# LanDiff/LanDiff

Measured on AMD Instinct MI355X. Metric: end-to-end frames/sec, 49f 480x720 @50 steps, higher is better.
Workload: dtype bf16; 1 GPU; LanDiff 5B full pipeline, single prompt per GPU, 49f 480x720, 50 sampler steps (VPSDE DPM-Solver++(2M), DynamicCFG), bf16, random-init weights at true shapes; frames=49, height=480, width=720, sampler_steps=50, llm_steps=1244, parallelism=dp1 over prompts, RCCL all_gather of uint8 frames only

## Files before the change

### landiff_amd/csrc/ld_llm.hip

```cpp
#include "ld_common.h"
#include "ld_llm_dev.h"
#include <stdio.h>
#include <stdlib.h>
#include "../../include/landiff_hip.h"

namespace {

constexpr int MAXB = 4;

struct GemvParams {
  const void* x;
  const void* W;
  const void* W2;
  const bf16_t* bias;
  const void* resid;
  void* out;
  int B, N, K;
  long ldx, ldo, ldr;
  int x_f32, w_f32, out_f32;
  int in_act, act;
  const float* norm_w;
  float norm_eps;
  ChainSync cs;
};
// ... 215 lines not shown
  constexpr int NV = R * B * (GATED ? 2 : 1), V = ceil_pow2(NV), LOGV = ilog2(V);
  constexpr int XAUX = CHAIN ? 16 : 0;
  __shared__ float red[2][4][V];
  __shared__ float ssq[4][B];

  const int tid = threadIdx.x, lane = tid & 63, wave = tid >> 6;
  const int nchunk = p.K >> 3;
  const int er = tid / B, eb = tid - er * B;

  u32x4_t wn[R][J], w2n[GATED ? R : 1][J];
  uint32_t e_bias_n = 0u, e_res_n = 0u;
  auto request = [&](int batch) {
    const int n0 = batch * R;
#pragma unroll
    for (int r = 0; r < R; ++r) {
      const long row = (n0 + r < p.N) ? n0 + r : p.N - 1;
#pragma unroll
      for (int j = 0; j < J; ++j) {
        const int c = j * 256 + tid;
        wn[r][j] = (u32x4_t){0u, 0u, 0u, 0u};
        if (c < nchunk) wn[r][j] = __builtin_nontemporal_load((const u32x4_t*)((const bf16_t*)p.W + row * p.K + c * 8));
        if (GATED) {
          w2n[r][j] = (u32x4_t){0u, 0u, 0u, 0u};
          if (c < nchunk) w2n[r][j] = __builtin_nontemporal_load((const u32x4_t*)((const bf16_t*)p.W2 + row * p.K + c * 8));
        }
      }
    }
    const int en = n0 + er;
    if (tid < R * B && en < p.N) {
      if (p.bias) e_bias_n = p.bias[en];
      if (p.resid) {
        if (CHAIN) e_res_n = __hip_atomic_load((const bf16_t*)p.resid + eb * p.ldr + en, __ATOMIC_RELAXED, __HIP_MEMORY_SCOPE_AGENT);
        else e_res_n = p.out_f32 ? ((const uint32_t*)p.resid)[eb * p.ldr + en] : (uint32_t)((const bf16_t*)p.resid)[eb * p.ldr + en];
      }
    }
  };

  u32x4_t xq[B][J];
  f32x4_t g0[NORM ? J : 1], g1[NORM ? J : 1];
  int batch = blockIdx.x;
  if (CHAIN) {
    request(batch);
    chain_wait(p.cs, tid);
  }
#pragma unroll
  for (int b = 0; b < B; ++b) {
    const __amdgpu_buffer_rsrc_t rx = __builtin_amdgcn_make_buffer_rsrc((void*)((const bf16_t*)p.x + b * p.ldx), 0, p.K * 2, 0x00020000);
#pragma unroll
    for (int j = 0; j < J; ++j) xq[b][j] = __builtin_amdgcn_raw_buffer_load_b128(rx, (j * 256 + tid) * 16, 0, XAUX);
  }
  if (NORM) {
    const __amdgpu_buffer_rsrc_t rg = __builtin_amdgcn_make_buffer_rsrc((void*)p.norm_w, 0, p.K * 4, 0x00020000);
#pragma unroll
    for (int j = 0; j < J; ++j) {
      const u32x4_t a = __builtin_amdgcn_raw_buffer_load_b128(rg, (j * 256 + tid) * 32, 0, 0);
      const u32x4_t b = __builtin_amdgcn_raw_buffer_load_b128(rg, (j * 256 + tid) * 32 + 16, 0, 0);
      g0[j] = __builtin_bit_cast(f32x4_t, a); g1[j] = __builtin_bit_cast(f32x4_t, b);
    }
  }
  if (!CHAIN) request(batch);

  if (NORM) {
#pragma unroll
    for (int b = 0; b < B; ++b) {
      const float ss = wave_sum(chunks_sumsq<J>(xq[b]));
      if (lane == 0) ssq[wave][b] = ss;
    }
    __syncthreads();
#pragma unroll
    for (int b = 0; b < B; ++b) {
      const float r1 = rsqrtf((ssq[0][b] + ssq[1][b] + ssq[2][b] + ssq[3][b]) / (float)p.K + p.norm_eps);
#pragma unroll
      for (int j = 0; j < J; ++j) {
        if (j * 256 + tid < nchunk) {
          const u32x4_t a = xq[b][j];
          xq[b][j] = (u32x4_t){pack_bf16x2(bf_lo(a[0]) * r1 * g0[j][0], bf_hi(a[0]) * r1 * g0[j][1]),
                               pack_bf16x2(bf_lo(a[1]) * r1 * g0[j][2], bf_hi(a[1]) * r1 * g0[j][3]),
                               pack_bf16x2(bf_lo(a[2]) * r1 * g1[j][0], bf_hi(a[2]) * r1 * g1[j][1]),
                               pack_bf16x2(bf_lo(a[3]) * r1 * g1[j][2], bf_hi(a[3]) * r1 * g1[j][3])};
        }
      }
    }
  }

  int par = 0;
#pragma unroll 1
  for (; batch < nbatch; batch += gridDim.x, par ^= 1) {
    u32x4_t w[R][J], w2[GATED ? R : 1][J];
#pragma unroll
    for (int r = 0; r < R; ++r)
#pragma unroll
      for (int j = 0; j < J; ++j) { w[r][j] = wn[r][j]; if (GATED) w2[r][j] = w2n[r][j]; }
    const uint32_t e_bias_raw = e_bias_n, e_res_raw = e_res_n;
    if (batch + (int)gridDim.x < nbatch) request(batch + gridDim.x);

    float v[V];
#pragma unroll
    for (int i = 0; i < V; ++i) v[i] = 0.f;
#pragma unroll
    for (int r = 0; r < R; ++r)
#pragma unroll
      for (int j = 0; j < J; ++j)
#pragma unroll
        for (int b = 0; b < B; ++b)
#pragma unroll
          for (int e = 0; e < 4; ++e) {
            v[r * B + b] = dot2_bf16(w[r][j][e], xq[b][j][e], v[r * B + b]);
            if (GATED) v[R * B + r * B + b] = dot2_bf16(w2[r][j][e], xq[b][j][e], v[R * B + r * B + b]);
          }
    wave_sum_multi<V>(v, lane);
    if ((lane & ((64 >> LOGV) - 1)) == 0) red[par][wave][lane >> (6 - LOGV)] = v[0];
    __syncthreads();
    const int en = batch * R + er;
    if (tid < R * B && en < p.N) {
      const float(&rd)[4][V] = red[par];
      float a = rd[0][tid] + rd[1][tid] + rd[2][tid] + rd[3][tid];
      const float e_bias = bf2f((bf16_t)e_bias_raw), e_res = p.out_f32 ? __uint_as_float(e_res_raw) : bf2f((bf16_t)e_res_raw);
      if (p.bias) a += e_bias;
      a = rbf(a);
      if (p.act) a = rbf(apply_act(p.act, a));
      if (GATED) a = rbf(a * rbf(rd[0][R * B + tid] + rd[1][R * B + tid] + rd[2][R * B + tid] + rd[3][R * B + tid]));
      if (p.resid) a = p.out_f32 ? e_res + a : rbf(e_res + a);
      if (CHAIN) __hip_atomic_store((bf16_t*)p.out + eb * p.ldo + en, f2bf(a), __ATOMIC_RELAXED, __HIP_MEMORY_SCOPE_AGENT);
      else if (p.out_f32) ((float*)p.out)[eb * p.ldo + en] = a;
      else ((bf16_t*)p.out)[eb * p.ldo + en] = f2bf(a);
    }
  }
  if (CHAIN) chain_arrive(p.cs, tid, blockIdx.x);
}

__global__ __launch_bounds__(256) void ld_rmsnorm_kernel(const bf16_t* x, const float* w, bf16_t* out,
                                                         int rows, int D, float eps) {
  const int lane = threadIdx.x & 63;
  const int r = blockIdx.x * 4 + (threadIdx.x >> 6);
  if (r >= rows) return;
  const bf16_t* xr = x + (long)r * D;
  float ss = 0.f;
  for (int c = lane; c < (D >> 3); c += 64) {
    const u32x4_t a = *(const u32x4_t*)(xr + c * 8);
#pragma unroll
    for (int e = 0; e < 4; ++e) { const float lo = bf_lo(a[e]), hi = bf_hi(a[e]); ss += lo * lo + hi * hi; }
  }
  ss = wave_sum(ss);
  const float rs = rsqrtf(ss / (float)D + eps);
  for (int c = lane; c < (D >> 3); c += 64) {
    const u32x4_t a = *(const u32x4_t*)(xr + c * 8);
    const f32x4_t w0 = *(const f32x4_t*)(w + c * 8), w1 = *(const f32x4_t*)(w + c * 8 + 4);
    float v[8];
#pragma unroll
    for (int e = 0; e < 4; ++e) { v[2 * e] = bf_lo(a[e]) * rs; v[2 * e + 1] = bf_hi(a[e]) * rs; }
    u32x4_t o;
    o[0] = pack_bf16x2(v[0] * w0[0], v[1] * w0[1]); o[1] = pack_bf16x2(v[2] * w0[2], v[3] * w0[3]);
    o[2] = pack_bf16x2(v[4] * w1[0], v[5] * w1[1]); o[3] = pack_bf16x2(v[6] * w1[2], v[7] * w1[3]);
    *(u32x4_t*)(out + (long)r * D + c * 8) = o;
  }
}

__global__ __launch_bounds__(256) void ld_ln_f32out_kernel(const bf16_t* x, long ldx, const float* w, const float* b,
                                                           float* out, int rows, int D, float eps) {
  const int lane = threadIdx.x & 63;
  const int r = blockIdx.x * 4 + (threadIdx.x >> 6);
  if (r >= rows) return;
  const bf16_t* xr = x + (long)r * ldx;
  float s = 0.f, ss = 0.f;
  for (int i = lane; i < D; i += 64) { const float v = bf2f(xr[i]); s += v; }
  s = wave_sum(s);
  const float mean = s / (float)D;
  for (int i = lane; i < D; i += 64) { const float d = bf2f(xr[i]) - mean; ss += d * d; }
  ss = wave_sum(ss);
  const float rs = rsqrtf(ss / (float)D + eps);
  for (int i = lane; i < D; i += 64) out[(long)r * D + i] = (bf2f(xr[i]) - mean) * rs * w[i] + b[i];
}

__global__ __launch_bounds__(256) void ld_ln_f32out_reg_kernel(const bf16_t* x, long ldx, const float* w, const float* b,
                                                               float* out, int rows, int D, float eps) {
  const int lane = threadIdx.x & 63;
  const int r = blockIdx.x * 4 + (threadIdx.x >> 6);
  if (r >= rows) return;
  const bf16_t* xr = x + (long)r * ldx;
  const int nchunk = D >> 3;
  float v[8][8];
  float s = 0.f, ss = 0.f;
#pragma unroll
  for (int k = 0; k < 8; ++k) {
    const int c = lane + 64 * k;
    u32x4_t a = (u32x4_t){0u, 0u, 0u, 0u};
    if (c < nchunk) a = *(const u32x4_t*)(xr + c * 8);
#pragma unroll
    for (int e = 0; e < 4; ++e) { v[k][2 * e] = bf_lo(a[e]); v[k][2 * e + 1] = bf_hi(a[e]); s += v[k][2 * e] + v[k][2 * e + 1]; }
  }
  s = wave_sum(s);
  const float mean = s / (float)D;
#pragma unroll
  for (int k = 0; k < 8; ++k) {
    if (lane + 64 * k < nchunk) {
#pragma unroll
      for (int e = 0; e < 8; ++e) { const float d = v[k][e] - mean; ss += d * d; }
    }
  }
  ss = wave_sum(ss);
  const float rs = rsqrtf(ss / (float)D + eps);
#pragma unroll
  for (int k = 0; k < 8; ++k) {
    const int c = lane + 64 * k;
    if (c < nchunk) {
      const f32x4_t w0 = *(const f32x4_t*)(w + c * 8), w1 = *(const f32x4_t*)(w + c * 8 + 4);
      const f32x4_t b0 = *(const f32x4_t*)(b + c * 8), b1 = *(const f32x4_t*)(b + c * 8 + 4);
      f32x4_t o0, o1;
#pragma unroll
      for (int e = 0; e < 4; ++e) { o0[e] = (v[k][e] - mean) * rs * w0[e] + b0[e]; o1[e] = (v[k][4 + e] - mean) * rs * w1[e] + b1[e]; }
      *(f32x4_t*)(out + (long)r * D + c * 8) = o0;
      *(f32x4_t*)(out + (long)r * D + c * 8 + 4) = o1;
    }
  }
}

__global__ void ld_rope_append_kernel(const bf16_t* qkv, const float* cos_t, const float* sin_t, const int* pos_ptr,
                                      bf16_t* q_out, bf16_t* kc, bf16_t* vc, int B, int m, int H, int Lmax) {
  const int D = 128;
  const int idx = blockIdx.x * blockDim.x + threadIdx.x;
  const int total = B * m * H * (D / 2);
  if (idx >= total) return;
  const int pr = idx % (D / 2);
  const int h = (idx / (D / 2)) % H;
  const int j = (idx / (D / 2) / H) % m;
  const int b = idx / (D / 2) / H / m;
  const int pos = *pos_ptr + j;
  const float c = cos_t[pos * (D / 2) + pr], s = sin_t[pos * (D / 2) + pr];
  const long base = (((long)(b * m + j) * 3) * H + h) * D + 2 * pr;
  const long hd = (long)H * D;
  const float qa = bf2f(qkv[base]), qb = bf2f(qkv[base + 1]);
  const float ka = bf2f(qkv[base + hd]), kb = bf2f(qkv[base + hd + 1]);
  const long qo = ((long)(b * m + j) * H + h) * D + 2 * pr;
  q_out[qo] = f2bf(qa * c - qb * s);
  q_out[qo + 1] = f2bf(qa * s + qb * c);
  const long co = (((long)b * Lmax + pos) * H + h) * D + 2 * pr;
  kc[co] = f2bf(ka * c - kb * s);
  kc[co + 1] = f2bf(ka * s + kb * c);
  vc[co] = qkv[base + 2 * hd];
  vc[co + 1] = qkv[base + 2 * hd + 1];
}

__global__ __launch_bounds__(256) void ld_kv_attn_kernel(const bf16_t* q, const bf16_t* kc, const bf16_t* vc,
                                                         const int* pos_ptr, bf16_t* out, int B, int m, int H, int Lmax) {
  extern __shared__ float sc[];
  const int D = 128;
  const int bh = blockIdx.x, j = blockIdx.y;
  const int b = bh / H, h = bh - b * H;
  const int L = *pos_ptr + j + 1;
  const int tid = threadIdx.x, lane = tid & 63, wave = tid >> 6;
  const bf16_t* qv = q + ((long)(b * m + j) * H + h) * D;
  const int sub = lane & 15, kq = lane >> 4;
  float qreg[8];
  {
    const u32x4_t a = *(const u32x4_t*)(qv + sub * 8);
#pragma unroll
    for (int e = 0; e < 4; ++e) { qreg[2 * e] = bf_lo(a[e]); qreg[2 * e + 1] = bf_hi(a[e]); }
  }
  const float inv_sqrt_d = 0.08838834764831845f;
  float lmax = -3.0e38f;
  for (int k0 = wave * 4; k0 < L; k0 += 16) {
    const int key = k0 + kq;
    float d = 0.f;
    if (key < L) {
      const u32x4_t a = *(const u32x4_t*)(kc + (((long)b * Lmax + key) * H + h) * D + sub * 8);
#pragma unroll
      for (int e = 0; e < 4; ++e) { d = fmaf(qreg[2 * e], bf_lo(a[e]), d); d = fmaf(qreg[2 * e + 1], bf_hi(a[e]), d); }
    }
    d += __shfl_xor(d, 1, 64); d += __shfl_xor(d, 2, 64); d += __shfl_xor(d, 4, 64); d += __shfl_xor(d, 8, 64);
    if (key < L) {
      const float s = rbf(rbf(d) * inv_sqrt_d);
      if (sub == 0) sc[key] = s;
      lmax = fmaxf(lmax, s);
    }
  }
  float* red = sc + Lmax;
  lmax = wave_max(lmax);
  if (lane == 0) red[wave] = lmax;
  __syncthreads();
  const float mx = fmaxf(fmaxf(red[0], red[1]), fmaxf(red[2], red[3]));
  float lsum = 0.f;
  for (int k = tid; k < L; k += 256) { const float e = __expf(sc[k] - mx); sc[k] = e; lsum += e; }
  lsum = wave_sum(lsum);
  __syncthreads();
  if (lane == 0) red[4 + wave] = lsum;
  __syncthreads();
  const float inv = 1.0f / (red[4] + red[5] + red[6] + red[7]);
  const int d = tid & 127, par = tid >> 7;
  float acc = 0.f;
  for (int k = par; k < L; k += 2) {
    const float pk = rbf(sc[k] * inv);
    acc = fmaf(pk, bf2f(vc[(((long)b * Lmax + k) * H + h) * D + d]), acc);
  }
  float* part = red + 8;
  part[par * 128 + d] = acc;
  __syncthreads();
  if (tid < 128) out[((long)(b * m + j) * H + h) * D + tid] = f2bf(part[tid] + part[128 + tid]);
}

__device__ __forceinline__ float ld_agent(const float* p) { return __hip_atomic_load(p, __ATOMIC_RELAXED, __HIP_MEMORY_SCOPE_AGENT); }
__device__ __forceinline__ void st_agent(float* p, float v) { __hip_atomic_store(p, v, __ATOMIC_RELAXED, __HIP_MEMORY_SCOPE_AGENT); }

template <bool CHAIN>
__global__ __launch_bounds__(256, CHAIN ? 2 : 1) void ld_kv_attn_split_kernel(const bf16_t* q, const bf16_t* qkv, const float* cos_t,
                                                               const float* sin_t, bf16_t* kc, bf16_t* vc,
                                                               const int* pos_ptr, int pos_value, float* ws, unsigned* counters,
                                                               bf16_t* out, int B, int H, int Lmax, int nsplit, KvSplitRule rule,
                                                               ChainSync cs) {
  __shared__ float red[8 + 4 * 128];
  __shared__ int is_last;
  const int D = 128;
  const int bh = blockIdx.x, sp = blockIdx.y;
  const int b = bh / H, h = bh - b * H;
  const int L = (pos_value >= 0 ? pos_value : *pos_ptr) + 1;
  const int ns = kv_eff_splits(L, nsplit, rule);
  const int tid = threadIdx.x, lane = tid & 63, wave = tid >> 6;
  if (sp >= ns) {
    if (CHAIN) { chain_wait(cs, tid); chain_arrive(cs, tid, blockIdx.y * gridDim.x + blockIdx.x); }
    return;
  }
  const int chunk = (L + ns - 1) / ns;
  const int k_begin = sp * chunk, k_end = min(L, k_begin + chunk);
  const int n = max(0, k_end - k_begin);
  const int sub = lane & 15, kq = lane >> 4;
  float* out_ws = ws + ((long)bh * nsplit + sp) * (D + 2);
  bf16_t* direct = (ns == 1 && !CHAIN) ? out + (long)bh * D : nullptr;
  KvRows rows;
  if (CHAIN) {
    if (n > 0) kv_rows_request(rows, kc, vc, (long)b * Lmax + k_begin, H, h, n, wave, kq, sub);
    chain_wait(cs, tid);
  }
  if (n == 0) {
    if (tid < D) st_agent(out_ws + 2 + tid, 0.f);
    if (tid == 0) { st_agent(out_ws, -3.0e38f); st_agent(out_ws + 1, 0.f); }
  } else {
    u32x4_t a_q = (u32x4_t){0u, 0u, 0u, 0u}, a_k = a_q, a_v = a_q;
    float cs_[4] = {0.f, 0.f, 0.f, 0.f}, sn[4] = {0.f, 0.f, 0.f, 0.f};
    const int pos = L - 1;
    if (qkv) {
      const bf16_t* src = qkv + ((long)b * 3 * H + h) * D;
      if (CHAIN) {
        const __amdgpu_buffer_rsrc_t rq = __builtin_amdgcn_make_buffer_rsrc((void*)src, 0, (2 * H + 1) * D * 2, 0x00020000);
        a_q = __builtin_amdgcn_raw_buffer_load_b128(rq, sub * 16, 0, 16);
        a_k = __builtin_amdgcn_raw_buffer_load_b128(rq, (H * D + sub * 8) * 2, 0, 16);
        a_v = __builtin_amdgcn_raw_buffer_load_b128(rq, (2 * H * D + sub * 8) * 2, 0, 16);
      } else {
        a_q = *(const u32x4_t*)(src + sub * 8);
        a_k = *(const u32x4_t*)(src + (long)H * D + sub * 8);
        a_v = *(const u32x4_t*)(src + 2L * H * D + sub * 8);
      }
#pragma unroll
      for (int e = 0; e < 4; ++e) { cs_[e] = cos_t[pos * 64 + sub * 4 + e]; sn[e] = sin_t[pos * 64 + sub * 4 + e]; }
    } else {
      a_q = *(const u32x4_t*)(q + ((long)b * H + h) * D + sub * 8);
    }
    if (!CHAIN) kv_rows_request(rows, kc, vc, (long)b * Lmax + k_begin, H, h, n, wave, kq, sub);
    kv_attn_split_core(rows, a_q, a_k, a_v, cs_, sn, qkv != nullptr, kc, vc, (long)b * Lmax + pos, H, h, pos - k_begin, n, true,
                       out_ws, red, red + 8, tid, lane, wave, [](float* p, float v) { st_agent(p, v); }, direct);
  }
  if (direct) return;
  asm volatile("s_waitcnt vmcnt(0)" ::: "memory");
  __syncthreads();
  if (tid == 0)
    is_last = __hip_atomic_fetch_add(counters + bh, 1u, __ATOMIC_RELAXED, __HIP_MEMORY_SCOPE_AGENT) == (unsigned)(ns - 1);
  __syncthreads();
  if (is_last) {
    if (tid < D) {
      const float r = kv_attn_combine_core(ws + (long)bh * nsplit * (D + 2), ns, tid, [](const float* p) { return ld_agent(p); });
      if (CHAIN) __hip_atomic_store(out + (long)bh * D + tid, f2bf(r), __ATOMIC_RELAXED, __HIP_MEMORY_SCOPE_AGENT);
      else out[(long)bh * D + tid] = f2bf(r);
    }
    if (tid == 0) __hip_atomic_store(counters + bh, 0u, __ATOMIC_RELAXED, __HIP_MEMORY_SCOPE_AGENT);
  }
  if (CHAIN) chain_arrive(cs, tid, blockIdx.y * gridDim.x + blockIdx.x);
}

__global__ void ld_embed_kernel(const float* table, const long* token, bf16_t* out, int B, int D) {
  const int i = blockIdx.x * blockDim.x + threadIdx.x;
  if (i >= B * D) return;
  const long t = *token;
  out[i] = f2bf(table[t * D + (i % D)]);
}

__global__ void ld_embed_pairs_kernel(const float* table, const long* token, bf16_t* out, int B, int D) {
  const int i = blockIdx.x * blockDim.x + threadIdx.x;
  if (i >= B * D) return;
  const long t = token[(i / D) >> 1];
  out[i] = f2bf(table[t * D + (i % D)]);
}

#define LD_SAMPLE_MAXV 4096
__device__ __forceinline__ float block_sum_1024(float v, float* red, int tid, int nthreads) {
  v = wave_sum(v);
  __syncthreads();
  if ((tid & 63) == 0) red[tid >> 6] = v;
  __syncthreads();
  float tot = 0.f;
  for (int w = 0; w < (nthreads >> 6); ++w) tot += red[w];
  return tot;
}
struct SampleArgs {
  const float* noise;
  const int* forced; int* pos; long* token; long* out_tokens; int* out_count; long* sampled;
  const float* emb; bf16_t* x; int B, D;
  long out_stride;
};
template <bool SAMPLE>
__global__ __launch_bounds__(1024) void ld_logits_to_probs_kernel(const float* logits, float* probs, float* cfg_logits,
                                                                  int V, int guided, float scale, float temperature,
                                                                  const int* pos_ptr, const int* allowed, int n_allowed_stride,
                                                                  int top_k, float top_p, SampleArgs sa) {
  __shared__ float red[32];
  __shared__ int redi[32];
  __shared__ float sv[LD_SAMPLE_MAXV];
  __shared__ float ss[LD_SAMPLE_MAXV];
  __shared__ float thr_s;
  const int tid = threadIdx.x, nt = blockDim.x;
  if constexpr (SAMPLE) {
    if (const long wg = blockIdx.x) {
      logits += wg * 2 * V; pos_ptr += wg;
      if (probs) probs += wg * V;
      if (cfg_logits) cfg_logits += wg * V;
      sa.noise += wg * V; sa.pos += wg; sa.token += wg; sa.out_tokens += wg * sa.out_stride; sa.out_count += wg;
      if (sa.sampled) sa.sampled += wg;
      sa.x += wg * sa.B * sa.D;
    }
  }
  const int* al = nullptr;
  int nal = 0;
  if (allowed) {
    al = allowed + (long)(*pos_ptr + 1) * n_allowed_stride;
    nal = al[0];
  }
  for (int i = tid; i < V; i += nt) {
    float l = logits[i];
    if (guided) { const float u = logits[V + i]; l = u + scale * (l - u); }
    if (cfg_logits) cfg_logits[i] = l;
    l = l / temperature;
    if (nal > 0) {
      bool ok = false;
      for (int a = 0; a < nal; ++a) ok |= (al[1 + a] == i);
      if (!ok) l = -INFINITY;
    }
    sv[i] = l;
  }
  __syncthreads();
  if (top_k > 0 && top_k < V && nal == 0) {
    for (int i = tid; i < V; i += nt) {
      const float v = sv[i];
      int gt = 0, ge = 0;
      for (int j = 0; j < V; ++j) { const float o = sv[j]; gt += (o > v); ge += (o >= v); }
      if (gt < top_k && top_k <= ge) thr_s = v;
    }
    __syncthreads();
    const float thr = thr_s;
    for (int i = tid; i < V; i += nt) if (sv[i] < thr) sv[i] = -INFINITY;
    __syncthreads();
  }
  float mx = -3.0e38f;
  for (int i = tid; i < V; i += nt) mx = fmaxf(mx, sv[i]);
  mx = wave_max(mx);
  if ((tid & 63) == 0) red[tid >> 6] = mx;
  __syncthreads();
  float m2 = red[0];
  for (int w = 1; w < (nt >> 6); ++w) m2 = fmaxf(m2, red[w]);
  float s = 0.f;
  for (int i = tid; i < V; i += nt) { const float e = expf(sv[i] - m2); sv[i] = e; s += e; }
  const float tot = block_sum_1024(s, red, tid, nt);
  for (int i = tid; i < V; i += nt) sv[i] = sv[i] / tot;
  __syncthreads();
  if (top_p >= 0.f && nal == 0) {
    int rk[(LD_SAMPLE_MAXV + 1023) / 1024];
    int c = 0;
    for (int i = tid; i < V; i += nt, ++c) {
      const float v = sv[i];
      int r = 0;
      for (int j = 0; j < V; ++j) { const float o = sv[j]; r += (o > v) || (o == v && j < i); }
      rk[c] = r;
      ss[r] = v;
    }
    __syncthreads();
    if (tid == 0) {
      float acc = 0.f;
      for (int j = 0; j < V; ++j) { acc += ss[j]; ss[j] = acc; }
    }
    __syncthreads();
    float ks = 0.f;
    c = 0;
    for (int i = tid; i < V; i += nt, ++c) {
      const int r = rk[c];
      if (r >= 1 && ss[r - 1] >= top_p) sv[i] = 0.f;
      ks += sv[i];
    }
    const float kept = block_sum_1024(ks, red, tid, nt);
    for (int i = tid; i < V; i += nt) sv[i] = sv[i] / kept;
    __syncthreads();
  }
  for (int i = tid; i < V; i += nt) if (probs) probs[i] = sv[i];
  if constexpr (SAMPLE) {
    float best = -INFINITY; int bi = 0x7fffffff;
    for (int i = tid; i < V; i += nt) {
      const float r = sv[i] / sa.noise[i];
      if (r > best || (r == best && i < bi) || bi == 0x7fffffff) { best = r; bi = i; }
    }
#pragma unroll
    for (int o = 32; o > 0; o >>= 1) {
      const float ob = __shfl_xor(best, o, 64); const int oi = __shfl_xor(bi, o, 64);
      if (ob > best || (ob == best && oi < bi)) { best = ob; bi = oi; }
    }
    __syncthreads();
    if ((tid & 63) == 0) { red[tid >> 6] = best; redi[tid >> 6] = bi; }
    __syncthreads();
    if (tid == 0) {
      for (int w = 1; w < (nt >> 6); ++w)
        if (red[w] > best || (red[w] == best && redi[w] < bi)) { best = red[w]; bi = redi[w]; }
      const int pos = *sa.pos;
      const int f = sa.forced[pos + 1];
      long t = bi;
      if (sa.sampled) *sa.sampled = t;
      if (f >= 0) t = f;
      else { sa.out_tokens[*sa.out_count] = t; *sa.out_count = *sa.out_count + 1; }
      *sa.token = t;
      *sa.pos = pos + 1;
      redi[0] = (int)t;
    }
    __syncthreads();
    const long t = redi[0];
    for (int i = tid; i < sa.B * sa.D; i += nt) sa.x[i] = f2bf(sa.emb[t * sa.D + (i % sa.D)]);
  }
}

__global__ void ld_decode_advance_kernel(const long* sampled, const int* forced, int* pos_ptr, long* token,
                                         long* out_tokens, int* out_count) {
  const int pos = *pos_ptr;
  const int f = forced[pos + 1];
  long t = *sampled;
  if (f >= 0) t = f;
  else { out_tokens[*out_count] = t; *out_count = *out_count + 1; }
  *token = t;
  *pos_ptr = pos + 1;
}

template <int B, bool WF32, int R, int U = 4>
int launch_gemv_cfg(const GemvParams& p, hipStream_t st) {
  const size_t smem = (size_t)B * p.K * (WF32 ? 4 : 2) + 64;
  static thread_local LdSmemCache cache{};
  if (int rc = ld_ensure_dyn_smem((const void*)ld_gemv_kernel<B, WF32, R, U>, smem, &cache)) return rc;
  long blocks = (p.N + 4 * R - 1) / (4 * R);
  if (blocks > 512) blocks = 512;
  hipLaunchKernelGGL((ld_gemv_kernel<B, WF32, R, U>), dim3((unsigned)blocks), dim3(256), smem, st, p);
  return ld_check_launch("ld_gemv");
}

template <int B, int R, int J, bool GATED, bool NORM>
int launch_gemv_reg(const GemvParams& p, hipStream_t st) {
  static const int cap = getenv("LD_GEMV_WGS") ? atoi(getenv("LD_GEMV_WGS")) : 768;
  const int nbatch = (p.N + R - 1) / R;
  const int trips = (nbatch + cap - 1) / cap;
  const int grid = (nbatch + trips - 1) / trips;
  hipLaunchKernelGGL((ld_gemv_reg_kernel<B, R, J, GATED, NORM>), dim3((unsigned)grid), dim3(256), 0, st, p, nbatch);
  return ld_check_launch("ld_gemv");
}

template <int B, int J, bool GATED, bool NORM>
int launch_gemv_reg_r(const GemvParams& p, int R, hipStream_t st) {
  constexpr int L1 = J * (GATED ? 2 : 1);
  if constexpr (L1 <= 2 && B <= 2) { if (R >= 8) return launch_gemv_reg<B, 8, J, GATED, NORM>(p, st); }
  if constexpr (L1 <= 4) { if (R >= 4) return launch_gemv_reg<B, 4, J, GATED, NORM>(p, st); }
  if (R >= 2) return launch_gemv_reg<B, 2, J, GATED, NORM>(p, st);
  return launch_gemv_reg<B, 1, J, GATED, NORM>(p, st);
}

template <int B, int J>
int launch_gemv_reg_j(const GemvParams& p, int R, hipStream_t st) {
  const bool gated = p.W2 != nullptr, norm = p.norm_w != nullptr;
  if constexpr (J <= 2) {
    if (gated) return norm ? launch_gemv_reg_r<B, J, true, true>(p, R, st) : launch_gemv_reg_r<B, J, true, false>(p, R, st);
  }
  return norm ? launch_gemv_reg_r<B, J, false, true>(p, R, st) : launch_gemv_reg_r<B, J, false, false>(p, R, st);
}

int gemv_mode() {
  static const int mode = getenv("LD_GEMV_MODE") ? atoi(getenv("LD_GEMV_MODE")) : 0;
  return mode;
}

int gemv_pair_reg_j(const GemvParams& p) {
  const int nchunk = p.K >> 3;
  if (gemv_mode() == 1 || p.w_f32 || p.x_f32 || p.in_act) return 0;
  if (nchunk <= 256) return 1;
  if (nchunk <= 512) return 2;
  if (nchunk <= 1536 && !p.W2) return 6;
  return 0;
}

template <int B>
int launch_gemv_pairs_b(const GemvParams& p, int J, hipStream_t st) {
  const bool gated = p.W2 != nullptr, norm = p.norm_w != nullptr;
  if (J == 1) {
    if (gated) return norm ? launch_gemv_reg<B, 4, 1, true, true>(p, st) : launch_gemv_reg<B, 4, 1, true, false>(p, st);
    return norm ? launch_gemv_reg<B, 4, 1, false, true>(p, st) : launch_gemv_reg<B, 4, 1, false, false>(p, st);
  }
  if (J == 2) {
    if (gated) return norm ? launch_gemv_reg<B, 2, 2, true, true>(p, st) : launch_gemv_reg<B, 2, 2, true, false>(p, st);
    return norm ? launch_gemv_reg<B, 4, 2, false, true>(p, st) : launch_gemv_reg<B, 4, 2, false, false>(p, st);
  }
  constexpr int R6 = B <= 4 ? 2 : 1;
  if constexpr (B <= 4) { if (norm) return launch_gemv_reg<B, R6, 6, false, true>(p, st); }
  return launch_gemv_reg<B, R6, 6, false, false>(p, st);
}

bool gemv_pairs_in_one_launch(const GemvParams& p, int J) { return p.B > 2 && J != 0 && !(J == 6 && p.norm_w && p.B > 4); }

template <int B>
int launch_gemv_b(const GemvParams& p, hipStream_t st) {
  const int mode = gemv_mode();
  static const int forced_r = getenv("LD_GEMV_R") ? atoi(getenv("LD_GEMV_R")) : 0;
  const int nchunk = p.K >> 3;
  const bool gated = p.W2 != nullptr;
  if (mode != 1 && !p.w_f32 && !p.x_f32 && !p.in_act) {
    if (nchunk <= 256) return launch_gemv_reg_j<B, 1>(p, forced_r ? forced_r : 4, st);
    if (nchunk <= 512) return launch_gemv_reg_j<B, 2>(p, forced_r ? forced_r : (gated ? 2 : 4), st);
    if constexpr (B <= 2) {
      if (nchunk <= 1536 && !gated) return launch_gemv_reg_j<B, 6>(p, forced_r ? forced_r : 2, st);
    }
  }
  if (p.w_f32) return launch_gemv_cfg<B, true, 1>(p, st);
  if (!p.W2 && nchunk <= 64 && p.N >= 4096) return launch_gemv_cfg<B, false, 8, 1>(p, st);
  if (p.W2 || p.N < 4096) return launch_gemv_cfg<B, false, 1>(p, st);
  return launch_gemv_cfg<B, false, 2>(p, st);
}

}

KvSplitRule ld_kv_split_rule() {
  static const KvSplitRule rule = [] {
    KvSplitRule r{KV_SPLIT_T1, KV_SPLIT_T2, KV_SPLIT_T4};
    if (const char* e = getenv("LD_KV_SPLIT_T")) {
      int a = 0, b = 0, c = 0;
      if (sscanf(e, "%d,%d,%d", &a, &b, &c) == 3) r = KvSplitRule{a, b, c};
    }
    return r;
  }();
  return rule;
}

LD_API int ld_gemv(const void* x, int64_t ldx, int32_t x_f32, const void* W, const void* W2, int32_t w_f32,
                   const void* bias, const void* resid, int64_t ldr, void* out, int64_t ldo, int32_t out_f32,
                   int64_t B, int64_t N, int64_t K, int32_t in_act, int32_t act, const float* norm_w, float norm_eps,
                   void* stream) {
  LD_REQUIRE(x && W && out, "ld_gemv: null pointer");
  LD_REQUIRE(B >= 1 && B <= MAXB, "ld_gemv: batch %ld not in [1,%d]", (long)B, MAXB);
  LD_REQUIRE(K % 8 == 0 && ldx % 8 == 0, "ld_gemv: K and ldx must be multiples of 8");
  LD_REQUIRE((size_t)B * K * (w_f32 ? 4 : 2) + 64 <= 160 * 1024, "ld_gemv: B*K too large for the LDS-staged activations");
  LD_REQUIRE(!(w_f32 && W2), "ld_gemv: gated form needs bf16 weights");
  LD_REQUIRE(!w_f32 || (x_f32 && out_f32), "ld_gemv: fp32 weights need fp32 in/out");
  GemvParams p{};
  p.x = x; p.W = W; p.W2 = W2; p.bias = (const bf16_t*)bias; p.resid = resid; p.out = out;
  p.B = (int)B; p.N = (int)N; p.K = (int)K; p.ldx = ldx; p.ldo = ldo; p.ldr = ldr;
  p.x_f32 = x_f32; p.w_f32 = w_f32; p.out_f32 = out_f32; p.in_act = in_act; p.act = act;
  p.norm_w = norm_w; p.norm_eps = norm_eps;
// ... 330 lines not shown
```

### landiff_amd/csrc/ld_llm_dev.h

```cpp
#pragma once
#include "ld_common.h"

typedef __attribute__((ext_vector_type(2))) __bf16 bf16x2_t;

__device__ __forceinline__ float dot2_bf16(uint32_t a, uint32_t b, float c) {
  return __builtin_amdgcn_fdot2_f32_bf16(__builtin_bit_cast(bf16x2_t, a), __builtin_bit_cast(bf16x2_t, b), c, false);
}

template <int V, int N = V, int O = 32>
__device__ __forceinline__ void wave_sum_multi(float (&v)[V], int lane) {
  if constexpr (N > 1) {
    const bool up = (lane & O) != 0;
#pragma unroll
    for (int i = 0; i < N / 2; ++i) {
      const float keep = up ? v[i + N / 2] : v[i];
      const float send = up ? v[i] : v[i + N / 2];
      v[i] = keep + __shfl_xor(send, O, 64);
    }
    wave_sum_multi<V, N / 2, O / 2>(v, lane);
  } else if constexpr (O > 0) {
    v[0] += __shfl_xor(v[0], O, 64);
    wave_sum_multi<V, 1, O / 2>(v, lane);
  }
}
constexpr int ceil_pow2(int v) { int p = 1; while (p < v) p <<= 1; return p; }
constexpr int ilog2(int v) { int l = 0; while ((1 << l) < v) ++l; return l; }

template <int J>
__device__ __forceinline__ float chunks_sumsq(const u32x4_t (&x)[J]) {
  float ss = 0.f;
#pragma unroll
  for (int j = 0; j < J; ++j)
#pragma unroll
    for (int e = 0; e < 4; ++e) { const float lo = bf_lo(x[j][e]), hi = bf_hi(x[j][e]); ss += lo * lo + hi * hi; }
  return ss;
}

constexpr int KV_MAXIT = 16;
struct KvRows { u32x4_t k[KV_MAXIT], v[KV_MAXIT]; };

struct KvSplitRule { int t1, t2, t4; };
constexpr int KV_SPLIT_T1 = 112, KV_SPLIT_T2 = 112, KV_SPLIT_T4 = 232;
__host__ __device__ inline int kv_eff_splits(int L, int nsplit_max, KvSplitRule r) {
  int ns = L <= r.t1 ? 1 : L <= r.t2 ? 2 : L <= r.t4 ? 4 : nsplit_max;
  if (ns > nsplit_max) ns = nsplit_max;
  while ((L + ns - 1) / ns > 16 * KV_MAXIT && ns < nsplit_max) ns = 2 * ns < nsplit_max ? 2 * ns : nsplit_max;
  return ns;
}
KvSplitRule ld_kv_split_rule();

__device__ __forceinline__ void kv_rows_request(KvRows& r, const bf16_t* kc, const bf16_t* vc, long row0, int H, int h, int n,
                                                int wave, int kq, int sub) {
#pragma unroll
  for (int it = 0; it < KV_MAXIT; ++it) {
    const int kk = wave * 4 + it * 16 + kq;
    r.k[it] = (u32x4_t){0u, 0u, 0u, 0u}; r.v[it] = (u32x4_t){0u, 0u, 0u, 0u};
    if (it * 16 >= n) continue;
    if (kk < n) {
      const long off = ((row0 + kk) * H + h) * 128 + sub * 8;
      r.k[it] = __builtin_nontemporal_load((const u32x4_t*)(kc + off));
      r.v[it] = __builtin_nontemporal_load((const u32x4_t*)(vc + off));
    }
  }
}

template <class Store>
__device__ __forceinline__ void kv_attn_split_core(KvRows& r, u32x4_t a_q, u32x4_t a_k, u32x4_t a_v, const float (&cs)[4],
                                                   const float (&sn)[4], bool rope, bf16_t* kc, bf16_t* vc, long cache_row,
                                                   int H, int h, int pk, int n, bool active, float* out_ws, float* red,
                                                   float* part, int t, int lane, int wave, Store store, bf16_t* direct_out = nullptr) {
  constexpr int D = 128;
  const int sub = lane & 15, kq = lane >> 4;
  float qreg[8];
  if (rope) {
    u32x4_t knew;
#pragma unroll
    for (int e = 0; e < 4; ++e) {
      const float qa = bf_lo(a_q[e]), qb = bf_hi(a_q[e]);
      qreg[2 * e] = rbf(qa * cs[e] - qb * sn[e]);
      qreg[2 * e + 1] = rbf(qa * sn[e] + qb * cs[e]);
      const float ka = bf_lo(a_k[e]), kb = bf_hi(a_k[e]);
      knew[e] = pack_bf16x2(ka * cs[e] - kb * sn[e], ka * sn[e] + kb * cs[e]);
    }
    if (active && pk >= 0 && pk < n) {
      if (wave == 0 && kq == 0) {
        const long co = (cache_row * H + h) * D + sub * 8;
        *(u32x4_t*)(kc + co) = knew;
        *(u32x4_t*)(vc + co) = a_v;
      }
#pragma unroll
      for (int it = 0; it < KV_MAXIT; ++it) {
        if (wave * 4 + it * 16 + kq == pk) { r.k[it] = knew; r.v[it] = a_v; }
      }
    }
  } else {
#pragma unroll
    for (int e = 0; e < 4; ++e) { qreg[2 * e] = bf_lo(a_q[e]); qreg[2 * e + 1] = bf_hi(a_q[e]); }
  }
  const float inv_sqrt_d = 0.08838834764831845f;
  float lmax = -3.0e38f;
  float sreg[KV_MAXIT];
#pragma unroll
  for (int it = 0; it < KV_MAXIT; ++it) {
    const int kk = wave * 4 + it * 16 + kq;
    sreg[it] = -3.0e38f;
    if (it * 16 >= n) continue;
    float d = 0.f;
#pragma unroll
    for (int e = 0; e < 4; ++e) { d = fmaf(qreg[2 * e], bf_lo(r.k[it][e]), d); d = fmaf(qreg[2 * e + 1], bf_hi(r.k[it][e]), d); }
    d += __shfl_xor(d, 1, 64); d += __shfl_xor(d, 2, 64); d += __shfl_xor(d, 4, 64); d += __shfl_xor(d, 8, 64);
    if (kk < n) {
      sreg[it] = rbf(rbf(d) * inv_sqrt_d);
      lmax = fmaxf(lmax, sreg[it]);
    }
  }
  lmax = wave_max(lmax);
  if (lane == 0) red[wave] = lmax;
  __syncthreads();
  const float mx = fmaxf(fmaxf(red[0], red[1]), fmaxf(red[2], red[3]));
  float acc[8];
#pragma unroll
  for (int e = 0; e < 8; ++e) acc[e] = 0.f;
  float lsum = 0.f;
#pragma unroll
  for (int it = 0; it < KV_MAXIT; ++it) {
    const int kk = wave * 4 + it * 16 + kq;
    if (it * 16 >= n) continue;
    if (kk < n) {
      const float pk_ = __expf(sreg[it] - mx);
      if (sub == 0) lsum += pk_;
#pragma unroll
      for (int e = 0; e < 4; ++e) { acc[2 * e] = fmaf(pk_, bf_lo(r.v[it][e]), acc[2 * e]); acc[2 * e + 1] = fmaf(pk_, bf_hi(r.v[it][e]), acc[2 * e + 1]); }
    }
  }
#pragma unroll
  for (int e = 0; e < 8; ++e) { acc[e] += __shfl_xor(acc[e], 16, 64); acc[e] += __shfl_xor(acc[e], 32, 64); }
  lsum = wave_sum(lsum);
  __syncthreads();
  if (kq == 0) {
#pragma unroll
    for (int e = 0; e < 8; ++e) part[wave * D + sub * 8 + e] = acc[e];
  }
  if (lane == 0) red[4 + wave] = lsum;
  __syncthreads();
  if (active) {
    if (direct_out) {
      if (t < D) direct_out[t] = f2bf((part[t] + part[D + t] + part[2 * D + t] + part[3 * D + t]) / (red[4] + red[5] + red[6] + red[7]));
    } else {
      if (t < D) store(out_ws + 2 + t, part[t] + part[D + t] + part[2 * D + t] + part[3 * D + t]);
      if (t == 0) { store(out_ws, mx); store(out_ws + 1, red[4] + red[5] + red[6] + red[7]); }
    }
  }
}

template <class Load>
__device__ __forceinline__ float kv_attn_combine_core(const float* w, int nsplit, int d, Load load) {
  constexpr int D = 128, U = 8;
  float mx = -3.0e38f;
  for (int s0 = 0; s0 < nsplit; s0 += U) {
    float m[U];
#pragma unroll
    for (int i = 0; i < U; ++i) m[i] = (s0 + i < nsplit) ? load(w + (s0 + i) * (D + 2)) : -3.0e38f;
#pragma unroll
    for (int i = 0; i < U; ++i) mx = fmaxf(mx, m[i]);
  }
  float l = 0.f, o = 0.f;
  for (int s0 = 0; s0 < nsplit; s0 += U) {
    float m[U], ls[U], os[U];
#pragma unroll
    for (int i = 0; i < U; ++i) {
      const bool live = s0 + i < nsplit;
      const float* ws = w + (s0 + i) * (D + 2);
      m[i] = live ? load(ws) : 0.f; ls[i] = live ? load(ws + 1) : 0.f; os[i] = live ? load(ws + 2 + d) : 0.f;
    }
#pragma unroll
    for (int i = 0; i < U; ++i) {
      if (s0 + i < nsplit) {
        const float f = __expf(m[i] - mx);
        l += f * ls[i];
        o += f * os[i];
      }
    }
  }
  return o / l;
}

struct ChainSync {
  unsigned* ctl;
  int slot;
  int prev_grid;
  unsigned epoch1;
};
constexpr int CHAIN_CTR0 = 64, CHAIN_CSTRIDE = 16, CHAIN_NCTR = 8;
constexpr unsigned CHAIN_SPIN_LIMIT = 1u << 20;

__device__ __forceinline__ void chain_wait(const ChainSync& cs, int tid) {
  if (cs.prev_grid > 0 && tid < 64) {
    const unsigned* ctr = cs.ctl + CHAIN_CTR0 + (cs.slot - 1) * CHAIN_NCTR * CHAIN_CSTRIDE;
    const unsigned mine = tid < CHAIN_NCTR ? cs.epoch1 * (unsigned)((cs.prev_grid - tid + CHAIN_NCTR - 1) / CHAIN_NCTR) : 0u;
    unsigned spins = 0;
    while (true) {
      const unsigned v = tid < CHAIN_NCTR ? __hip_atomic_load(ctr + tid * CHAIN_CSTRIDE, __ATOMIC_RELAXED, __HIP_MEMORY_SCOPE_AGENT) : 0u;
      if (__builtin_amdgcn_ballot_w64(v < mine) == 0) break;
      if ((spins & 63) == 63 && __hip_atomic_load(cs.ctl, __ATOMIC_RELAXED, __HIP_MEMORY_SCOPE_AGENT) != 0) break;
      __builtin_amdgcn_s_sleep(1);
      if (++spins > CHAIN_SPIN_LIMIT) {
        if (tid == 0) __hip_atomic_store(cs.ctl, 1u, __ATOMIC_RELAXED, __HIP_MEMORY_SCOPE_AGENT);
        break;
      }
    }
  }
  __syncthreads();
}

__device__ __forceinline__ void chain_arrive(const ChainSync& cs, int tid, int wg) {
  asm volatile("s_waitcnt vmcnt(0)" ::: "memory");
  __syncthreads();
  if (tid == 0)
    __hip_atomic_fetch_add(cs.ctl + CHAIN_CTR0 + (cs.slot * CHAIN_NCTR + (wg & (CHAIN_NCTR - 1))) * CHAIN_CSTRIDE, 1u, __ATOMIC_RELAXED,
                           __HIP_MEMORY_SCOPE_AGENT);
}
```

Before: 3.094 frames/s.

## Stage KV loads through buffer loads to cut registers in split-KV decode attention

The non-chained split-KV decode attention kernel now uses a new staged core. It loads K rows with raw buffer loads, and for long splits it reuses the K registers to fetch V after each score is computed, so it no longer holds full K and V arrays at once. Short splits use a half-size variant. The kernel is now always compiled with launch bounds for two blocks per CU to raise occupancy. The cost is that V loads are serialized behind the score computation, and the register cap may cause spills.

```diff
diff --git a/landiff_amd/csrc/ld_llm.hip b/landiff_amd/csrc/ld_llm.hip
--- a/landiff_amd/csrc/ld_llm.hip
+++ b/landiff_amd/csrc/ld_llm.hip
@@ -541,7 +541,7 @@
 __device__ __forceinline__ void st_agent(float* p, float v) { __hip_atomic_store(p, v, __ATOMIC_RELAXED, __HIP_MEMORY_SCOPE_AGENT); }
 
 template <bool CHAIN>
-__global__ __launch_bounds__(256, CHAIN ? 2 : 1) void ld_kv_attn_split_kernel(const bf16_t* q, const bf16_t* qkv, const float* cos_t,
+__global__ __launch_bounds__(256, 2) void ld_kv_attn_split_kernel(const bf16_t* q, const bf16_t* qkv, const float* cos_t,
                                                                const float* sin_t, bf16_t* kc, bf16_t* vc,
                                                                const int* pos_ptr, int pos_value, float* ws, unsigned* counters,
                                                                bf16_t* out, int B, int H, int Lmax, int nsplit, KvSplitRule rule,
@@ -593,9 +593,17 @@
     } else {
       a_q = *(const u32x4_t*)(q + ((long)b * H + h) * D + sub * 8);
     }
-    if (!CHAIN) kv_rows_request(rows, kc, vc, (long)b * Lmax + k_begin, H, h, n, wave, kq, sub);
-    kv_attn_split_core(rows, a_q, a_k, a_v, cs_, sn, qkv != nullptr, kc, vc, (long)b * Lmax + pos, H, h, pos - k_begin, n, true,
-                       out_ws, red, red + 8, tid, lane, wave, [](float* p, float v) { st_agent(p, v); }, direct);
+    if constexpr (CHAIN)
+      kv_attn_split_core(rows, a_q, a_k, a_v, cs_, sn, qkv != nullptr, kc, vc, (long)b * Lmax + pos, H, h, pos - k_begin, n, true,
+                         out_ws, red, red + 8, tid, lane, wave, [](float* p, float v) { st_agent(p, v); }, direct);
+    else if (n <= 16 * (KV_MAXIT / 2))
+      kv_attn_split_core_staged<KV_MAXIT / 2, false>(a_q, a_k, a_v, cs_, sn, qkv != nullptr, kc, vc, (long)b * Lmax + k_begin,
+                                                     (long)b * Lmax + pos, H, h, pos - k_begin, n, out_ws, red, red + 8, tid, lane, wave,
+                                                     [](float* p, float v) { st_agent(p, v); }, direct);
+    else
+      kv_attn_split_core_staged<KV_MAXIT, true>(a_q, a_k, a_v, cs_, sn, qkv != nullptr, kc, vc, (long)b * Lmax + k_begin,
+                                                (long)b * Lmax + pos, H, h, pos - k_begin, n, out_ws, red, red + 8, tid, lane, wave,
+                                                [](float* p, float v) { st_agent(p, v); }, direct);
   }
   if (direct) return;
   asm volatile("s_waitcnt vmcnt(0)" ::: "memory");
diff --git a/landiff_amd/csrc/ld_llm_dev.h b/landiff_amd/csrc/ld_llm_dev.h
--- a/landiff_amd/csrc/ld_llm_dev.h
+++ b/landiff_amd/csrc/ld_llm_dev.h
@@ -60,6 +60,60 @@
       const long off = ((row0 + kk) * H + h) * 128 + sub * 8;
       r.k[it] = __builtin_nontemporal_load((const u32x4_t*)(kc + off));
       r.v[it] = __builtin_nontemporal_load((const u32x4_t*)(vc + off));
+    }
+  }
+}
+
+__device__ __forceinline__ void kv_new_token(u32x4_t a_q, u32x4_t a_k, const float (&cs)[4], const float (&sn)[4], bool rope,
+                                             float (&qreg)[8], u32x4_t& knew) {
+  knew = (u32x4_t){0u, 0u, 0u, 0u};
+  if (rope) {
+#pragma unroll
+    for (int e = 0; e < 4; ++e) {
+      const float qa = bf_lo(a_q[e]), qb = bf_hi(a_q[e]);
+      qreg[2 * e] = rbf(qa * cs[e] - qb * sn[e]);
+      qreg[2 * e + 1] = rbf(qa * sn[e] + qb * cs[e]);
+      const float ka = bf_lo(a_k[e]), kb = bf_hi(a_k[e]);
+      knew[e] = pack_bf16x2(ka * cs[e] - kb * sn[e], ka * sn[e] + kb * cs[e]);
+    }
+  } else {
+#pragma unroll
+    for (int e = 0; e < 4; ++e) { qreg[2 * e] = bf_lo(a_q[e]); qreg[2 * e + 1] = bf_hi(a_q[e]); }
+  }
+}
+__device__ __forceinline__ float kv_dot16(const float (&qreg)[8], u32x4_t k) {
+  float d = 0.f;
+#pragma unroll
+  for (int e = 0; e < 4; ++e) { d = fmaf(qreg[2 * e], bf_lo(k[e]), d); d = fmaf(qreg[2 * e + 1], bf_hi(k[e]), d); }
+  d += __shfl_xor(d, 1, 64); d += __shfl_xor(d, 2, 64); d += __shfl_xor(d, 4, 64); d += __shfl_xor(d, 8, 64);
+  return d;
+}
+__device__ __forceinline__ float kv_score(float d) { return rbf(rbf(d) * 0.08838834764831845f); }
+__device__ __forceinline__ void kv_pv(float (&acc)[8], float p, u32x4_t v) {
+#pragma unroll
+  for (int e = 0; e < 4; ++e) { acc[2 * e] = fmaf(p, bf_lo(v[e]), acc[2 * e]); acc[2 * e + 1] = fmaf(p, bf_hi(v[e]), acc[2 * e + 1]); }
+}
+template <class Store>
+__device__ __forceinline__ void kv_split_finish(float (&acc)[8], float lsum, float mx, bool active, float* out_ws, float* red,
+                                                float* part, int t, int lane, int wave, Store store, bf16_t* direct_out) {
+  constexpr int D = 128;
+  const int sub = lane & 15, kq = lane >> 4;
+#pragma unroll
+  for (int e = 0; e < 8; ++e) { acc[e] += __shfl_xor(acc[e], 16, 64); acc[e] += __shfl_xor(acc[e], 32, 64); }
+  lsum = wave_sum(lsum);
+  __syncthreads();
+  if (kq == 0) {
+#pragma unroll
+    for (int e = 0; e < 8; ++e) part[wave * D + sub * 8 + e] = acc[e];
+  }
+  if (lane == 0) red[4 + wave] = lsum;
+  __syncthreads();
+  if (active) {
+    if (direct_out) {
+      if (t < D) direct_out[t] = f2bf((part[t] + part[D + t] + part[2 * D + t] + part[3 * D + t]) / (red[4] + red[5] + red[6] + red[7]));
+    } else {
+      if (t < D) store(out_ws + 2 + t, part[t] + part[D + t] + part[2 * D + t] + part[3 * D + t]);
+      if (t == 0) { store(out_ws, mx); store(out_ws + 1, red[4] + red[5] + red[6] + red[7]); }
     }
   }
 }
@@ -72,32 +126,19 @@
   constexpr int D = 128;
   const int sub = lane & 15, kq = lane >> 4;
   float qreg[8];
-  if (rope) {
-    u32x4_t knew;
-#pragma unroll
-    for (int e = 0; e < 4; ++e) {
-      const float qa = bf_lo(a_q[e]), qb = bf_hi(a_q[e]);
-      qreg[2 * e] = rbf(qa * cs[e] - qb * sn[e]);
-      qreg[2 * e + 1] = rbf(qa * sn[e] + qb * cs[e]);
-      const float ka = bf_lo(a_k[e]), kb = bf_hi(a_k[e]);
-      knew[e] = pack_bf16x2(ka * cs[e] - kb * sn[e], ka * sn[e] + kb * cs[e]);
-    }
-    if (active && pk >= 0 && pk < n) {
-      if (wave == 0 && kq == 0) {
-        const long co = (cache_row * H + h) * D + sub * 8;
-        *(u32x4_t*)(kc + co) = knew;
-        *(u32x4_t*)(vc + co) = a_v;
-      }
-#pragma unroll
-      for (int it = 0; it < KV_MAXIT; ++it) {
-        if (wave * 4 + it * 16 + kq == pk) { r.k[it] = knew; r.v[it] = a_v; }
-      }
-    }
-  } else {
-#pragma unroll
-    for (int e = 0; e < 4; ++e) { qreg[2 * e] = bf_lo(a_q[e]); qreg[2 * e + 1] = bf_hi(a_q[e]); }
-  }
-  const float inv_sqrt_d = 0.08838834764831845f;
+  u32x4_t knew;
+  kv_new_token(a_q, a_k, cs, sn, rope, qreg, knew);
+  if (rope && active && pk >= 0 && pk < n) {
+    if (wave == 0 && kq == 0) {
+      const long co = (cache_row * H + h) * D + sub * 8;
+      *(u32x4_t*)(kc + co) = knew;
+      *(u32x4_t*)(vc + co) = a_v;
+    }
+#pragma unroll
+    for (int it = 0; it < KV_MAXIT; ++it) {
+      if (wave * 4 + it * 16 + kq == pk) { r.k[it] = knew; r.v[it] = a_v; }
+    }
+  }
   float lmax = -3.0e38f;
   float sreg[KV_MAXIT];
 #pragma unroll
@@ -105,12 +146,9 @@
     const int kk = wave * 4 + it * 16 + kq;
     sreg[it] = -3.0e38f;
     if (it * 16 >= n) continue;
-    float d = 0.f;
-#pragma unroll
-    for (int e = 0; e < 4; ++e) { d = fmaf(qreg[2 * e], bf_lo(r.k[it][e]), d); d = fmaf(qreg[2 * e + 1], bf_hi(r.k[it][e]), d); }
-    d += __shfl_xor(d, 1, 64); d += __shfl_xor(d, 2, 64); d += __shfl_xor(d, 4, 64); d += __shfl_xor(d, 8, 64);
-    if (kk < n) {
-      sreg[it] = rbf(rbf(d) * inv_sqrt_d);
+    const float d = kv_dot16(qreg, r.k[it]);
+    if (kk < n) {
+      sreg[it] = kv_score(d);
       lmax = fmaxf(lmax, sreg[it]);
     }
   }
@@ -129,28 +167,85 @@
     if (kk < n) {
       const float pk_ = __expf(sreg[it] - mx);
       if (sub == 0) lsum += pk_;
-#pragma unroll
-      for (int e = 0; e < 4; ++e) { acc[2 * e] = fmaf(pk_, bf_lo(r.v[it][e]), acc[2 * e]); acc[2 * e + 1] = fmaf(pk_, bf_hi(r.v[it][e]), acc[2 * e + 1]); }
-    }
-  }
-#pragma unroll
-  for (int e = 0; e < 8; ++e) { acc[e] += __shfl_xor(acc[e], 16, 64); acc[e] += __shfl_xor(acc[e], 32, 64); }
-  lsum = wave_sum(lsum);
-  __syncthreads();
-  if (kq == 0) {
-#pragma unroll
-    for (int e = 0; e < 8; ++e) part[wave * D + sub * 8 + e] = acc[e];
-  }
-  if (lane == 0) red[4 + wave] = lsum;
-  __syncthreads();
-  if (active) {
-    if (direct_out) {
-      if (t < D) direct_out[t] = f2bf((part[t] + part[D + t] + part[2 * D + t] + part[3 * D + t]) / (red[4] + red[5] + red[6] + red[7]));
-    } else {
-      if (t < D) store(out_ws + 2 + t, part[t] + part[D + t] + part[2 * D + t] + part[3 * D + t]);
-      if (t == 0) { store(out_ws, mx); store(out_ws + 1, red[4] + red[5] + red[6] + red[7]); }
-    }
-  }
+      kv_pv(acc, pk_, r.v[it]);
+    }
+  }
+  kv_split_finish(acc, lsum, mx, active, out_ws, red, part, t, lane, wave, store, direct_out);
+}
+
+template <int NIT, bool STAGED, class Store>
+__device__ __forceinline__ void kv_attn_split_core_staged(u32x4_t a_q, u32x4_t a_k, u32x4_t a_v, const float (&cs)[4],
+                                                          const float (&sn)[4], bool rope, bf16_t* kc, bf16_t* vc, long row0,
+                                                          long cache_row, int H, int h, int pk, int n, float* out_ws, float* red,
+                                                          float* part, int t, int lane, int wave, Store store, bf16_t* direct_out) {
+  constexpr int D = 128;
+  const int sub = lane & 15, kq = lane >> 4;
+  const long base = (row0 * H + h) * D;
+  const int stride = H * D * 2;
+  const int bytes = (n - 1) * stride + D * 2;
+  const __amdgpu_buffer_rsrc_t rk = __builtin_amdgcn_make_buffer_rsrc((void*)(kc + base), 0, bytes, 0x00020000);
+  const __amdgpu_buffer_rsrc_t rv = __builtin_amdgcn_make_buffer_rsrc((void*)(vc + base), 0, bytes, 0x00020000);
+  const int voff = (wave * 4 + kq) * stride + sub * 16;
+  constexpr int AUX_NT = 2;
+  u32x4_t kv[NIT], vv[STAGED ? 1 : NIT];
+#pragma unroll
+  for (int it = 0; it < NIT; ++it) {
+    kv[it] = (u32x4_t){0u, 0u, 0u, 0u};
+    if constexpr (!STAGED) vv[it] = (u32x4_t){0u, 0u, 0u, 0u};
+    if (it * 16 >= n) continue;
+    kv[it] = __builtin_amdgcn_raw_buffer_load_b128(rk, voff + it * 16 * stride, 0, AUX_NT);
+    if constexpr (!STAGED) vv[it] = __builtin_amdgcn_raw_buffer_load_b128(rv, voff + it * 16 * stride, 0, AUX_NT);
+  }
+  float qreg[8];
+  u32x4_t knew;
+  kv_new_token(a_q, a_k, cs, sn, rope, qreg, knew);
+  const bool here = rope && pk >= 0 && pk < n;
+  if (here && wave == 0 && kq == 0) {
+    const long co = (cache_row * H + h) * D + sub * 8;
+    *(u32x4_t*)(kc + co) = knew;
+    *(u32x4_t*)(vc + co) = a_v;
+  }
+  float lmax = -3.0e38f;
+  float sreg[NIT];
+#pragma unroll
+  for (int it = 0; it < NIT; ++it) {
+    const int kk = wave * 4 + it * 16 + kq;
+    sreg[it] = -3.0e38f;
+    if (it * 16 >= n) continue;
+    const bool mine = here && kk == pk;
+    u32x4_t k = kv[it];
+#pragma unroll
+    for (int e = 0; e < 4; ++e) k[e] = mine ? knew[e] : k[e];
+    const float d = kv_dot16(qreg, k);
+    if constexpr (STAGED) kv[it] = __builtin_amdgcn_raw_buffer_load_b128(rv, voff + it * 16 * stride, 0, AUX_NT);
+    if (kk < n) {
+      sreg[it] = kv_score(d);
+      lmax = fmaxf(lmax, sreg[it]);
+    }
+  }
+  lmax = wave_max(lmax);
+  if (lane == 0) red[wave] = lmax;
+  __syncthreads();
+  const float mx = fmaxf(fmaxf(red[0], red[1]), fmaxf(red[2], red[3]));
+  float acc[8];
+#pragma unroll
+  for (int e = 0; e < 8; ++e) acc[e] = 0.f;
+  float lsum = 0.f;
+#pragma unroll
+  for (int it = 0; it < NIT; ++it) {
+    const int kk = wave * 4 + it * 16 + kq;
+    if (it * 16 >= n) continue;
+    if (kk < n) {
+      const float pk_ = __expf(sreg[it] - mx);
+      if (sub == 0) lsum += pk_;
+      const bool mine = here && kk == pk;
+      u32x4_t v = STAGED ? kv[it] : vv[it];
+#pragma unroll
+      for (int e = 0; e < 4; ++e) v[e] = mine ? a_v[e] : v[e];
+      kv_pv(acc, pk_, v);
+    }
+  }
+  kv_split_finish(acc, lsum, mx, true, out_ws, red, part, t, lane, wave, store, direct_out);
 }
 
 template <class Load>
```

Result: no change. 3.097 frames/s, median of 6 (+0.1%).
